# carrenD/Medical-Cross-Modality-Domain-Adaptation

Hardware: AMD Instinct MI355X
Metric: training slices/sec (256x256x3, B=16/GPU) joint segmenter+GAN step (1 dis update on B MR + B CT, clip, 1 gen update on B CT) (higher is better)
Workload: dtype f32; 1 GPU; BASELINE configs[3]: train_gan.py --phase train-gan joint step, B=16/GPU per domain, f32, dropout .75, mask critic on; global_batch=16, per_gpu_batch=16, parallelism=dp1, step_capture=False

## Files before the change

include/pnp_hip.h:

```cpp
#ifndef PNP_HIP_H
#define PNP_HIP_H

#include <stddef.h>
#include <stdint.h>

#ifdef __cplusplus
extern "C" {
#endif

#define PNP_OK 0
#define PNP_EINVAL (-1)
#define PNP_ELAUNCH (-2)
#define PNP_EWORKSPACE (-3)
#define PNP_ECOMM (-4)

#define PNP_DTYPE_F32 0
#define PNP_DTYPE_BF16 1
#define PNP_DTYPE_F64 2

#define PNP_PAD_ZERO 0
#define PNP_PAD_SYMMETRIC 1

int pnp_abi_version(void);
const char* pnp_last_error(void);
int pnp_device_info(int device, int* cu_count, int* clock_khz, int* lds_bytes, char* arch, int arch_len);

#define PNP_PROF_CONV_FWD 1
#define PNP_PROF_CONV_DGRAD 2
#define PNP_PROF_CONV_WGRAD 4
#define PNP_PROF_CONV_DIRECT 8
typedef struct pnp_prof_row {
    char name[128];
    int64_t launches;
    double ms, flops, bytes;
} pnp_prof_row;
int pnp_prof_enable(int32_t mask);
int pnp_prof_summary(pnp_prof_row* rows, int32_t max_rows);

typedef struct pnp_conv_geom {
    int32_t N, H, W, C;
    int32_t K, R, S;
    int32_t OH, OW;
    int32_t stride, dil;
    int32_t pad_t, pad_l;
    int32_t pad_mode;
    int32_t dtype;
} pnp_conv_geom;

int pnp_conv2d_fwd(const float* x, const float* w, float* y, const pnp_conv_geom* g,
                   float keep_prob, uint64_t seed, uint32_t stream_id, void* stream);
size_t pnp_conv2d_fwd_workspace_bytes(const pnp_conv_geom* g);
int pnp_conv2d_fwd_ws(const float* x, const float* w, float* y, const pnp_conv_geom* g,
                      float keep_prob, uint64_t seed, uint32_t stream_id,
                      void* workspace, size_t workspace_bytes, void* stream);

int32_t pnp_conv2d_fwd_stats_parts(const pnp_conv_geom* g);
int pnp_conv2d_fwd_stats(const float* x, const float* w, float* y, const pnp_conv_geom* g,
                         float keep_prob, uint64_t seed, uint32_t stream_id,
                         const float* shift , float* parts, size_t parts_bytes, void* stream);
int32_t pnp_conv2d_fwd_stats_ws_parts(const pnp_conv_geom* g);
int pnp_conv2d_fwd_stats_ws(const float* x, const float* w, float* y, const pnp_conv_geom* g,
                            float keep_prob, uint64_t seed, uint32_t stream_id,
                            const float* shift , float* parts, size_t parts_bytes,
// ... 245 lines not shown
```

medical-cross-modality-domain-adaptation_amd/_lib.py:

```python
import ctypes
import os

import torch

from ctypes import POINTER, c_char_p, c_float, c_int, c_int32, c_int64, c_size_t, c_uint32, c_uint64, c_void_p

_HERE = os.path.dirname(os.path.abspath(__file__))
LIB_PATH = os.environ.get("PNP_LIB") or os.path.join(_HERE, "libpnp_hip.so")

PAD_ZERO = 0
PAD_SYMMETRIC = 1
OPT_CHUNK = 1024
DTYPE_F32, DTYPE_BF16, DTYPE_F64 = 0, 1, 2
COMM_ID_BYTES = 128
(ROUTE_IGEMM, ROUTE_N16, ROUTE_NARROW, ROUTE_WINO, ROUTE_X3D, ROUTE_X3S, ROUTE_PHASES,
 ROUTE_WINO_WGRAD, ROUTE_X3W, ROUTE_N16_WGRAD, ROUTE_WGD, ROUTE_RING) = range(12)
ABI_VERSION = 4


class ConvGeom(ctypes.Structure):
    _fields_ = [(n, c_int32) for n in
                ("N", "H", "W", "C", "K", "R", "S", "OH", "OW", "stride", "dil", "pad_t", "pad_l", "pad_mode", "dtype")]

    def key(self):
        return tuple(getattr(self, f) for f, _ in self._fields_)


class ProfRow(ctypes.Structure):
    _fields_ = [("name", ctypes.c_char * 128), ("launches", c_int64), ("ms", ctypes.c_double), ("flops", ctypes.c_double),
                ("bytes", ctypes.c_double)]


class AugVolume(ctypes.Structure):
    _fields_ = [("image", c_void_p), ("label", c_void_p), ("X", c_int32), ("Y", c_int32), ("Z", c_int32), ("fill", c_float)]


class AugSample(ctypes.Structure):
    _fields_ = [("volume", c_int32), ("frame", c_int32), ("m", c_float * 6)]


class AugSampleZ(ctypes.Structure):
    _fields_ = [("volume", c_int32), ("frame", c_int32), ("dz", c_float), ("m", c_float * 6)]


PROF_CONV_FWD, PROF_CONV_DGRAD, PROF_CONV_WGRAD, PROF_CONV_DIRECT = 1, 2, 4, 8


class PnpError(RuntimeError):
    pass


_F = c_void_p
_G = POINTER(ConvGeom)

PROTOTYPES = {
    "pnp_abi_version": (c_int, []),
    "pnp_last_error": (c_char_p, []),
    "pnp_device_info": (c_int, [c_int, POINTER(c_int), POINTER(c_int), POINTER(c_int), c_char_p, c_int]),
    "pnp_prof_enable": (c_int, [c_int32]),
    "pnp_prof_summary": (c_int, [POINTER(ProfRow), c_int32]),
    "pnp_conv2d_fwd": (c_int, [_F, _F, _F, _G, c_float, c_uint64, c_uint32, c_void_p]),
    "pnp_conv2d_dgrad_workspace_bytes": (c_size_t, [_G]),
    "pnp_conv2d_dgrad": (c_int, [_F, _F, _F, _G, c_void_p, c_size_t, c_void_p]),
    "pnp_conv2d_dgrad_add": (c_int, [_F, _F, _F, _F, _G, c_void_p, c_size_t, c_void_p]),
    "pnp_conv2d_wgrad_workspace_bytes": (c_size_t, [_G]),
    "pnp_conv2d_wgrad": (c_int, [_F, _F, _F, _G, c_void_p, c_size_t, c_void_p]),
    "pnp_conv2d_wgrad_acc": (c_int, [_F, _F, _F, _G, c_void_p, c_size_t, c_void_p]),
    "pnp_conv2d_fwd_workspace_bytes": (c_size_t, [_G]),
    "pnp_conv2d_fwd_ws": (c_int, [_F, _F, _F, _G, c_float, c_uint64, c_uint32, c_void_p, c_size_t, c_void_p]),
    "pnp_conv2d_fwd_stats_parts": (c_int32, [_G]),
    "pnp_conv2d_fwd_stats": (c_int, [_F, _F, _F, _G, c_float, c_uint64, c_uint32, _F, _F, c_size_t, c_void_p]),
    "pnp_bn_stats_finish": (c_int, [_F, c_int32, _F, _F, _F, _F, _F, c_int64, c_int32, c_float, c_void_p]),
    "pnp_bn_fold": (c_int, [_F, _F, _F, _F, _F, _F, c_int32, c_float, c_void_p]),
    "pnp_conv2d_fwd_bn": (c_int, [_F, _F, _F, _G, c_float, c_uint64, c_uint32, _F, _F, _F, c_int32, c_float, c_void_p]),
    "pnp_conv2d_fwd_bn_ws": (c_int, [_F, _F, _F, _G, c_float, c_uint64, c_uint32, _F, _F, _F, c_int32, c_float, c_void_p, c_size_t, c_void_p]),
    "pnp_conv2d_fwd_stats_ws_parts": (c_int32, [_G]),
    "pnp_conv2d_fwd_stats_ws": (c_int, [_F, _F, _F, _G, c_float, c_uint64, c_uint32, _F, _F, c_size_t, c_void_p, c_size_t, c_void_p]),
    "pnp_conv2d_wino_chosen": (c_int32, [_G, c_int32]),
# ... 151 lines not shown
```

medical-cross-modality-domain-adaptation_amd/csrc/conv_wino.hip:

```cpp
#include <atomic>
#include <map>
#include <mutex>
#include "conv_common.h"
#include "conv_mma.h"

using namespace pnpconv;

namespace {

constexpr int NT = 256;

__device__ __forceinline__ f32x4 ld4(const float* p) { return *reinterpret_cast<const f32x4*>(p); }
__device__ __forceinline__ void st4(float* p, f32x4 v) { *reinterpret_cast<f32x4*>(p) = v; }

typedef __bf16 bf16x4 __attribute__((ext_vector_type(4)));
__device__ __forceinline__ void split3(float v, __bf16& hi, __bf16& mid, __bf16& lo) {
    hi = (__bf16)v;
    const float r = v - (float)hi;
    mid = (__bf16)r;
    lo = (__bf16)(r - (float)mid);
}
__device__ __forceinline__ void st4x3(__bf16* p, size_t pstride, f32x4 v) {
    bf16x4 h, m, l;
#pragma unroll
// ... 387 lines not shown
#pragma unroll
        for (int i = 0; i < NR; ++i) abase[i] = abase_n[i];
#pragma unroll
        for (int i = 0; i < NPB; ++i) boff[i] = boff_n[i];
        pos = pos_n; m0 = m0_n; n0 = n0_n;
        if (next_tail) in_tail = true;
        else local = nl;
    }
}

struct WinoOutArgs {
    const float* Mm;
    float* y;
    WinoGeom g;
    int K;
    int tiles_per_block;
    int do_drop;
    uint32_t drop_thresh, drop_key;
    float drop_keep;
    const pnp_step_params* sp;
    uint32_t drop_sid;
    const float* res_add;
    float* stat_ws;
    const float* stat_shift;
    const float* ep_scale;
    const float* ep_shift;
    const float* ep_res;
    int ep_cs;
    float ep_alpha;
    const float* Px;
    int tail_P, tail_F, tail_R, tail_s, tail_bn, nblk_m, nblk_n, gn;
};

template <int M, bool TS = false>
__global__ void __launch_bounds__(NT) wino_out_kernel(WinoOutArgs a) {
    constexpr int P = M + 2;
    __shared__ float red[NT * 8];
    const int K4 = a.K >> 2;
    const int kq0 = blockIdx.y * NT;
    const int K4s = (K4 - kq0) < NT ? (K4 - kq0) : NT;
    const int rpi = NT / K4s;
    const int tid = threadIdx.x;
    const int cg = tid % K4s, rsub = tid / K4s;
    const bool active = rsub < rpi;
    const int k = (kq0 + cg) * 4;
    const int t0 = blockIdx.x * a.tiles_per_block;
    int t1 = t0 + a.tiles_per_block;
    if (t1 > a.g.T) t1 = a.g.T;
    const size_t plane = (size_t)a.g.T * a.K;
    const uint32_t dkey = a.do_drop ? pnp_eff_drop_key(a.drop_key, a.sp, a.drop_sid) : 0u;
    const bool stats = a.stat_ws != nullptr;
    f32x4 s0 = {0, 0, 0, 0}, s1 = {0, 0, 0, 0};
    if (active) {
        f32x4 shift = {0, 0, 0, 0}, sc = {0, 0, 0, 0}, sh = {0, 0, 0, 0};
        if (stats && a.stat_shift) shift = ld4(a.stat_shift + k);
        if (a.ep_scale) {
            sc = ld4(a.ep_scale + k);
            sh = ld4(a.ep_shift + k);
        }
        const int cpad = (a.K - a.ep_cs) >> 1;
        for (int t = t0 + rsub; t < t1; t += rpi) {
            int n, pa, pb, ti, tj;
            tile_of(a.g, t, n, pa, pb, ti, tj);
            const float* src = a.Mm + (size_t)t * a.K + k;
            f32x4 m[P][P];
#pragma unroll
            for (int p = 0; p < P; ++p)
#pragma unroll
                for (int q = 0; q < P; ++q) m[p][q] = ld4(src + (size_t)(P * p + q) * plane);
            if constexpr (TS) {
                const int mt = t >> 7, nt = k / a.tail_bn;
                int bid;
                if (a.gn <= 0 || a.gn >= a.nblk_n) bid = mt * a.nblk_n + nt;
                else {
                    const int sc = nt / a.gn, left = a.nblk_n - sc * a.gn;
                    const int width = left < a.gn ? left : a.gn;
                    bid = sc * (a.nblk_m * a.gn) + mt * width + (nt - sc * a.gn);
                }
                const int nblk = a.nblk_m * a.nblk_n;
                int x = bid / a.tail_P, local = bid - x * a.tail_P;
                const size_t tsz = (size_t)128 * a.tail_bn;
                const size_t inner = (size_t)(t & 127) * a.tail_bn + (k - nt * a.tail_bn);
#pragma unroll
                for (int p = 0; p < P; ++p)
#pragma unroll
                    for (int q = 0; q < P; ++q) {
                        if (local >= a.tail_F) {
                            const float* px = a.Px + (size_t)(x * a.tail_R + local - a.tail_F) * (a.tail_s - 1) * tsz + inner;
                            for (int pc = 0; pc < a.tail_s - 1; ++pc) m[p][q] += ld4(px + pc * tsz);
                        }
                        local += nblk;
                        if (local >= a.tail_P) {
                            local -= a.tail_P;
                            ++x;
                        }
                    }
            }
            f32x4 o[M][M];
            if constexpr (M == 2) {
                f32x4 r[2][4];
#pragma unroll
                for (int q = 0; q < 4; ++q) {
                    r[0][q] = m[0][q] + m[1][q] + m[2][q];
                    r[1][q] = m[1][q] - m[2][q] - m[3][q];
                }
#pragma unroll
                for (int p = 0; p < 2; ++p) {
                    o[p][0] = r[p][0] + r[p][1] + r[p][2];
                    o[p][1] = r[p][1] - r[p][2] - r[p][3];
                }
            } else {
                f32x4 r[4][6];
#pragma unroll
                for (int q = 0; q < 6; ++q) {
                    f32x4 c4[4];
                    w4_at(m[0][q], m[1][q], m[2][q], m[3][q], m[4][q], m[5][q], c4);
#pragma unroll
                    for (int p = 0; p < 4; ++p) r[p][q] = c4[p];
                }
#pragma unroll
                for (int p = 0; p < 4; ++p) w4_at(r[p][0], r[p][1], r[p][2], r[p][3], r[p][4], r[p][5], o[p]);
            }
#pragma unroll
            for (int p = 0; p < M; ++p)
#pragma unroll
                for (int q = 0; q < M; ++q) {
                    const int u = M * ti + p, v = M * tj + q;
                    if (u >= a.g.Hso || v >= a.g.Wso) continue;
                    const size_t row = (size_t)(n * a.g.Ho + pa + a.g.dil * u) * a.g.Wo + pb + a.g.dil * v;
                    const size_t idx = row * a.K + k;
                    f32x4 val = o[p][q];
                    if (a.do_drop) {
#pragma unroll
                        for (int e = 0; e < 4; ++e)
                            val[e] = pnp_drop_keep((uint32_t)(idx + e), dkey, a.drop_thresh) ? val[e] / a.drop_keep : 0.f;
                    }
                    if (a.res_add) val += ld4(a.res_add + idx);
                    if (stats) {
#pragma unroll
                        for (int e = 0; e < 4; ++e) {
                            const float d = val[e] - shift[e];
                            s0[e] += d;
                            s1[e] = fmaf(d, d, s1[e]);
                        }
                    }
                    if (a.ep_scale) {
#pragma unroll
                        for (int e = 0; e < 4; ++e) val[e] = fmaf(val[e], sc[e], sh[e]);
                        if (a.ep_res) {
#pragma unroll
                            for (int e = 0; e < 4; ++e) {
                                const int cs = k + e - cpad;
                                if ((unsigned)cs < (unsigned)a.ep_cs) val[e] += a.ep_res[row * a.ep_cs + cs];
                            }
                        }
                        if (a.ep_alpha >= 0.f) {
#pragma unroll
                            for (int e = 0; e < 4; ++e) val[e] = val[e] < 0.f ? val[e] * a.ep_alpha : val[e];
                        }
                    }
                    st4(a.y + idx, val);
                }
        }
    }
    if (!stats) return;
#pragma unroll
    for (int e = 0; e < 4; ++e) {
        red[tid * 8 + e] = s0[e];
        red[tid * 8 + 4 + e] = s1[e];
    }
    __syncthreads();
    if (tid < K4s) {
        f32x4 a0 = {0, 0, 0, 0}, a1 = {0, 0, 0, 0};
        for (int j = 0; j < rpi; ++j) {
            const int tt = j * K4s + tid;
#pragma unroll
            for (int e = 0; e < 4; ++e) {
                a0[e] += red[tt * 8 + e];
                a1[e] += red[tt * 8 + 4 + e];
            }
        }
        st4(a.stat_ws + ((size_t)blockIdx.x * 2 + 0) * a.K + k, a0);
        st4(a.stat_ws + ((size_t)blockIdx.x * 2 + 1) * a.K + k, a1);
    }
}


struct WinoDyArgs {
    const float* dy;
    float* Y;
    WinoGeom g;
    int K;
};

template <int M>
__global__ void __launch_bounds__(NT) wino_dy_kernel(WinoDyArgs a) {
    const int K4 = a.K >> 2;
    const size_t nvec = (size_t)a.g.T * K4;
    const size_t plane = (size_t)a.g.T * a.K;
    const size_t gs = (size_t)gridDim.x * NT;
    for (size_t i = (size_t)blockIdx.x * NT + threadIdx.x; i < nvec; i += gs) {
        const int t = (int)(i / K4);
        const int k = (int)(i - (size_t)t * K4) * 4;
        int n, pa, pb, ti, tj;
        tile_of(a.g, t, n, pa, pb, ti, tj);
        f32x4 y[M][M];
#pragma unroll
        for (int p = 0; p < M; ++p)
#pragma unroll
            for (int q = 0; q < M; ++q) {
                const int u = M * ti + p, v = M * tj + q;
                const f32x4 zero = {0, 0, 0, 0};
                y[p][q] = (u < a.g.Hso && v < a.g.Wso) ? ld4(a.dy + ((size_t)(n * a.g.Ho + pa + a.g.dil * u) * a.g.Wo + pb + a.g.dil * v) * a.K + k) : zero;
            }
        float* out = a.Y + (size_t)t * a.K + k;
        if constexpr (M == 2) {
// ... 639 lines not shown
        ga.V = V; ga.U = U; ga.Mm = Mm; ga.T = w.T; ga.C = a.C; ga.K = a.K;
        const bool narrow = a.K <= 64;
        ga.nblk_m = pnp_cdiv(w.T, 128); ga.nblk_n = pnp_cdiv(a.K, narrow ? 64 : 128);
        static const int wino_gn = env_int("PNP_WINO_GN", -1);
        ga.gn = wino_gn >= 0 ? wino_gn : a.gn; ga.xcd_swizzle = xcd ? 2 : 0;
        ga.npos = NP;
        ga.whole = ((double)NP * w.T * a.C * 4.0 < 2147483648.0 && (double)NP * a.C * a.K * 4.0 < 2147483648.0) ? 1 : 0;
        ga.tail_F = plan.F; ga.tail_R = plan.R; ga.tail_s = plan.s; ga.Px = Px;
        dim3 grid((unsigned)plan.grid);
        const double fl = 2.0 * NP * (double)w.T * a.C * a.K;
        const double by = 4.0 * NP * ((double)w.T * a.C + (double)a.C * a.K + (double)w.T * a.K);
        constexpr int KB = M == 4 ? 2 : 0;
        PnpProfScope ps(cls, st, fl, by, "wino_gemm_kernel<128, %d, 2, 2, %d>", narrow ? 64 : 128, KB + (kind != 0));
        if (narrow) {
            if (kind == 0) hipLaunchKernelGGL((wino_gemm_kernel<128, 64, 2, 2, KB>), grid, dim3(NTHREADS), 0, st, ga);
            else hipLaunchKernelGGL((wino_gemm_kernel<128, 64, 2, 2, KB + 1>), grid, dim3(NTHREADS), 0, st, ga);
        } else if (kind == 0) hipLaunchKernelGGL((wino_gemm_kernel<128, 128, 2, 2, KB>), grid, dim3(NTHREADS), 0, st, ga);
        else hipLaunchKernelGGL((wino_gemm_kernel<128, 128, 2, 2, KB + 1>), grid, dim3(NTHREADS), 0, st, ga);
        PNP_CHECK_LAUNCH("wino_gemm_kernel");
    }
    {
        WinoOutArgs oa{};
        oa.Mm = Mm; oa.y = a.y; oa.g = w; oa.K = a.K;
        int nblk;
        out_plan(w.T, a.K, &oa.tiles_per_block, &nblk);
        oa.do_drop = a.do_drop; oa.drop_thresh = a.drop_thresh; oa.drop_key = a.drop_key; oa.drop_keep = a.drop_keep;
        oa.sp = a.sp; oa.drop_sid = a.drop_sid;
        oa.res_add = a.res_add; oa.stat_ws = a.stat_ws; oa.stat_shift = a.stat_shift;
        oa.ep_scale = a.ep_scale; oa.ep_shift = a.ep_shift; oa.ep_res = a.ep_res; oa.ep_cs = a.ep_cs; oa.ep_alpha = a.ep_alpha;
        oa.Px = Px; oa.tail_P = plan.P; oa.tail_F = plan.F; oa.tail_R = plan.R; oa.tail_s = plan.s; oa.tail_bn = a.K <= 64 ? 64 : 128;
        static const int wino_gn_o = env_int("PNP_WINO_GN", -1);
        oa.nblk_m = pnp_cdiv(w.T, 128); oa.nblk_n = pnp_cdiv(a.K, oa.tail_bn); oa.gn = wino_gn_o >= 0 ? wino_gn_o : a.gn;
        dim3 grid((unsigned)nblk, (unsigned)pnp_cdiv(a.K / 4, NT));
        PnpProfScope ps(cls, st, 0.0, 4.0 * ((double)NP * w.T * a.K + (double)a.M * a.K), "wino_out_kernel<%d>", M);
        if (oa.tail_s > 1) hipLaunchKernelGGL((wino_out_kernel<M, true>), grid, dim3(NT), 0, st, oa);
        else hipLaunchKernelGGL((wino_out_kernel<M, false>), grid, dim3(NT), 0, st, oa);
        PNP_CHECK_LAUNCH("wino_out_kernel");
    }
    return PNP_OK;
}

int launch_wino(const ConvArgs& a, int kind, bool flip_transpose, void* ws, size_t ws_bytes, hipStream_t st) {
    const int m = plan_tile(a, false);
    PNP_REQUIRE(m == 2 || m == 4, "launch_wino: the planner does not route this layer (policy changed between the query and the launch?)");
    return m == 4 ? launch_wino_m<4>(a, kind, flip_transpose, ws, ws_bytes, st) : launch_wino_m<2>(a, kind, flip_transpose, ws, ws_bytes, st);
}

int wino_wgrad_tile(const pnp_conv_geom* g) { return plan_tile(g, true); }

inline int x3_tp(int T) { return (T + 63) & ~63; }
inline bool use_x3_wgrad(int T, int C, int K) {
    static const int on = env_int("PNP_WINOGRAD_X3_WGRAD", 1), tmin = env_int("PNP_WINOGRAD_X3_WGRAD_TMIN", 256), tmax = env_int("PNP_WINOGRAD_X3_WGRAD_TMAX", 2048);
    const int m = wino_x3_mode();
    if (!on || m == 0 || !wino_x3_dims_ok(C, x3_tp(T), K) || !wino_x3_dims_ok(K, x3_tp(T), C)) return false;
    return m >= 2 || (T >= tmin && T <= tmax);
}
int wgrad_split_x3(int T, int C, int K, int npos, int* sps) {
    const int nchunks = x3_tp(T) / 64;
    const long long tiles = (long long)pnp_cdiv(C, 128) * pnp_cdiv(K, K <= 64 ? 64 : 128) * npos;
    int best = 1;
    double best_cost = 1e30;
    for (int ns = 1; ns <= 32 && ns <= nchunks; ++ns) {
        const int cps = pnp_cdiv(nchunks, ns);
        if (pnp_cdiv(nchunks, cps) != ns) continue;
        if (ns > 1 && cps < 2) break;
        const int rounds = pnp_cdiv(tiles * ns, 256);
        const double cost = rounds * (2.0 * cps + 3.0) + ns * 1.5e-6 * npos * (double)C * K;
        if (cost < best_cost - 1e-9) { best_cost = cost; best = ns; }
    }
// ... 189 lines not shown
```

medical-cross-modality-domain-adaptation_amd/csrc/elementwise.hip:

```cpp
#include <atomic>
#include <mutex>
#include "pnp_common.h"

namespace {

constexpr int NT = 256;

__device__ __forceinline__ f32x4 ld4(const float* p) { return *reinterpret_cast<const f32x4*>(p); }
__device__ __forceinline__ void st4(float* p, f32x4 v) { *reinterpret_cast<f32x4*>(p) = v; }
typedef __bf16 bf16x4_t __attribute__((ext_vector_type(4)));
__device__ __forceinline__ void st4h(__bf16* p, f32x4 v) {
    bf16x4_t h;
    h[0] = (__bf16)v[0]; h[1] = (__bf16)v[1]; h[2] = (__bf16)v[2]; h[3] = (__bf16)v[3];
    *reinterpret_cast<bf16x4_t*>(p) = h;
}

inline dim3 grid_rows(long long P, int C4, int cap = 256 * 8) {
    const int ny = (C4 + NT - 1) / NT;
    const int c4s = C4 < NT ? C4 : NT;
    const int rpi = NT / c4s;
    long long bx = (P + rpi - 1) / rpi;
    const long long cx = cap / ny > 0 ? cap / ny : 1;
    if (bx > cx) bx = cx;
    if (bx < 1) bx = 1;
// ... 2 lines not shown

inline int grid_for(size_t nvec, int cap = 256 * 8) {
    long long b = (long long)((nvec + NT - 1) / NT);
    if (b > cap) b = cap;
    if (b < 1) b = 1;
    return (int)b;
}

struct ColArgs {
    const float* x;
    const float* dout;
    const float* out;
    const float* mean;
    const float* var;
    const float* gamma;
    const float* beta;
    float* ws;
    long long P;
    int C;
    int rows_per_block;
    float eps, alpha;
    unsigned* tick;
    int nslab;
    float* o0;
    float* o1;
    float* acc0;
    float* acc1;
    float* mm;
    float* mv;
    float decay;
};

constexpr int COLRED_SLAB = 128;

template <int KIND>
__global__ void __launch_bounds__(NT) colreduce_kernel(ColArgs a) {
    __shared__ float red[NT * 8];
    __shared__ int s_last;
    const int C4 = a.C >> 2;
    const int rpi = NT / C4;
    const int t = threadIdx.x;
    const int cg = t % C4, rsub = t / C4;
    const bool active = rsub < rpi;
    const long long r0 = (long long)blockIdx.x * a.rows_per_block;
    long long r1 = r0 + a.rows_per_block;
    if (r1 > a.P) r1 = a.P;
    f32x4 s0 = {0, 0, 0, 0}, s1 = {0, 0, 0, 0};
    if (active) {
        const int c = cg * 4;
        f32x4 m, rs, gsc = {0, 0, 0, 0}, bet = {0, 0, 0, 0};
        if constexpr (KIND == 0) {
            m = ld4(a.x + c);
        } else {
            m = ld4(a.mean + c);
            f32x4 v = ld4(a.var + c);
#pragma unroll
            for (int e = 0; e < 4; ++e) rs[e] = 1.0f / sqrtf(v[e] + a.eps);
            if (!a.out && a.alpha >= 0.f) {
                const f32x4 ga = ld4(a.gamma + c);
                bet = ld4(a.beta + c);
#pragma unroll
                for (int e = 0; e < 4; ++e) gsc[e] = ga[e] * rs[e];
            }
        }
        for (long long r = r0 + rsub; r < r1; r += rpi) {
            const size_t off = (size_t)r * a.C + c;
            f32x4 xv = ld4(a.x + off);
            if constexpr (KIND == 0) {
#pragma unroll
                for (int e = 0; e < 4; ++e) {
                    float d = xv[e] - m[e];
                    s0[e] += d;
                    s1[e] = fmaf(d, d, s1[e]);
                }
            } else {
                f32x4 g = ld4(a.dout + off);
                if (a.alpha >= 0.f) {
                    if (a.out) {
                        f32x4 o = ld4(a.out + off);
#pragma unroll
                        for (int e = 0; e < 4; ++e) g[e] = o[e] > 0.f ? g[e] : g[e] * a.alpha;
                    } else {
#pragma unroll
                        for (int e = 0; e < 4; ++e) g[e] = fmaf(xv[e] - m[e], gsc[e], bet[e]) > 0.f ? g[e] : g[e] * a.alpha;
                    }
                }
#pragma unroll
                for (int e = 0; e < 4; ++e) {
                    float xh = (xv[e] - m[e]) * rs[e];
                    s0[e] += g[e];
                    s1[e] = fmaf(g[e], xh, s1[e]);
                }
            }
        }
    }
#pragma unroll
    for (int e = 0; e < 4; ++e) {
        red[t * 8 + e] = s0[e];
        red[t * 8 + 4 + e] = s1[e];
    }
    __syncthreads();
    if (t < C4) {
        f32x4 a0 = {0, 0, 0, 0}, a1 = {0, 0, 0, 0};
        for (int j = 0; j < rpi; ++j) {
            const int tt = j * C4 + t;
#pragma unroll
            for (int e = 0; e < 4; ++e) {
                a0[e] += red[tt * 8 + e];
                a1[e] += red[tt * 8 + 4 + e];
            }
        }
        float* w0 = a.ws + ((size_t)blockIdx.x * 2 + 0) * a.C + t * 4;
        float* w1 = a.ws + ((size_t)blockIdx.x * 2 + 1) * a.C + t * 4;
        st4(w0, a0);
        st4(w1, a1);
    }
    if (!a.tick) return;
    const int nblk = (int)gridDim.x;
    const int slab = blockIdx.x / COLRED_SLAB;
    const int b0 = slab * COLRED_SLAB;
    const int b1 = (b0 + COLRED_SLAB < nblk) ? b0 + COLRED_SLAB : nblk;
    __threadfence();
    __syncthreads();
    if (t == 0) s_last = (atomicAdd(&a.tick[slab], 1u) == (unsigned)(b1 - b0 - 1));
    __syncthreads();
    if (!s_last) return;
    __threadfence();
    double* dred = reinterpret_cast<double*>(red);
    double d0[4] = {0, 0, 0, 0}, d1[4] = {0, 0, 0, 0};
    if (active) {
        for (int b = b0 + rsub; b < b1; b += rpi) {
            const f32x4 v0 = ld4(a.ws + ((size_t)b * 2 + 0) * a.C + cg * 4), v1 = ld4(a.ws + ((size_t)b * 2 + 1) * a.C + cg * 4);
#pragma unroll
            for (int e = 0; e < 4; ++e) {
                d0[e] += (double)v0[e];
                d1[e] += (double)v1[e];
            }
        }
    }
    double t0[4] = {0, 0, 0, 0}, t1[4] = {0, 0, 0, 0};
#pragma unroll
    for (int q = 0; q < 2; ++q) {
// ... 164 lines not shown
        s1 += red[1][j][cl];
    }
    if constexpr (KIND == 0) {
        const double inv = 1.0 / (double)P;
        const double md = s0 * inv;
        double var = s1 * inv - md * md;
        if (var < 0.0) var = 0.0;
        const float meanf = (float)((double)x0[c] + md), varf = (float)var;
        o0[c] = meanf;
        o1[c] = varf;
        if (mm) {
            const float one_minus = 1.0f - decay;
            const float bessel = P > 1 ? (float)((double)P / (double)(P - 1)) : 1.0f;
            mm[c] -= (mm[c] - meanf) * one_minus;
            mv[c] -= (mv[c] - varf * bessel) * one_minus;
        }
    } else {
        o0[c] = (float)s0;
        o1[c] = (float)s1;
        if (acc0) {
            acc0[c] += (float)s0;
            acc1[c] += (float)s1;
        }
    }
}

template <int KIND>
int launch_colreduce_final(float* ws, const float* x0, float* o0, float* o1, int nblk, int C, long long P, float* mm, float* mv, float decay,
                           hipStream_t st, const char* who, float* acc0 = nullptr, float* acc1 = nullptr) {
    static const int two_stage = getenv("PNP_BN_FINAL_1STAGE") ? 0 : 1;
    int slab = 0, n = nblk;
    if (two_stage && nblk >= 4 * COLRED_SLAB) {
        const int nslab = nblk / COLRED_SLAB;
        hipLaunchKernelGGL(colreduce_compact_kernel, dim3(pnp_cdiv(C, 32), nslab), dim3(1024), 0, st, ws, nblk, nslab, C);
        PNP_CHECK_LAUNCH(who);
        slab = COLRED_SLAB;
        n = 2 * nslab;
    }
    hipLaunchKernelGGL(colreduce_final_kernel<KIND>, dim3(pnp_cdiv(C, 32)), dim3(1024), 0, st, (const float*)ws, x0, o0, o1, n, C, P, mm, mv,
                       decay, slab, acc0, acc1);
    PNP_CHECK_LAUNCH(who);
    return PNP_OK;
}

int colreduce_plan(long long P, int C, int* nblk, int* rpb) {
    static const int cap = getenv("PNP_BN_NBLK") ? atoi(getenv("PNP_BN_NBLK")) : 2048;
    long long b = (P + 63) / 64;
    if (b > cap) b = cap;
    if (b < 1) b = 1;
    long long r = (P + b - 1) / b;
    b = (P + r - 1) / r;
    *nblk = (int)b;
    *rpb = (int)r;
    (void)C;
    return 0;
}

constexpr int TICKET_SLOTS = 512, TICKET_STRIDE = 32;
unsigned* ticket_slot(hipStream_t st, int nslab) {
    static const int on = getenv("PNP_BN_ONE_LAUNCH") ? atoi(getenv("PNP_BN_ONE_LAUNCH")) : 0;
    if (!on || nslab + 1 > TICKET_STRIDE) return nullptr;
    constexpr int MAXDEV = 16;
    static std::atomic<unsigned*> bufs[MAXDEV];
    static std::atomic<unsigned> seq{0};
    static std::mutex mx;
    int dev = 0;
    if (hipGetDevice(&dev) != hipSuccess || dev < 0 || dev >= MAXDEV) {
        (void)hipGetLastError();
        return nullptr;
    }
    std::atomic<unsigned*>& buf = bufs[dev];
    unsigned* b = buf.load(std::memory_order_acquire);
    if (!b) {
        hipStreamCaptureStatus cs = hipStreamCaptureStatusNone;
        if (hipStreamIsCapturing(st, &cs) != hipSuccess || cs != hipStreamCaptureStatusNone) {
            (void)hipGetLastError();
            return nullptr;
        }
        std::lock_guard<std::mutex> lk(mx);
        b = buf.load(std::memory_order_acquire);
        if (!b) {
            if (hipMalloc((void**)&b, sizeof(unsigned) * TICKET_SLOTS * TICKET_STRIDE) != hipSuccess ||
                hipMemset(b, 0, sizeof(unsigned) * TICKET_SLOTS * TICKET_STRIDE) != hipSuccess || hipDeviceSynchronize() != hipSuccess) {
                (void)hipGetLastError();
                return nullptr;
            }
            buf.store(b, std::memory_order_release);
        }
    }
    return b + (size_t)(seq.fetch_add(1, std::memory_order_relaxed) % TICKET_SLOTS) * TICKET_STRIDE;
}

template <int KIND>
int run_colreduce(ColArgs a, float* o0, float* o1, void* ws, size_t ws_bytes, hipStream_t st, const char* who, float* mm = nullptr,
                  float* mv = nullptr, float decay = 0.f, float* acc0 = nullptr, float* acc1 = nullptr) {
    int nblk, rpb;
    colreduce_plan(a.P, a.C, &nblk, &rpb);
    const size_t need = (size_t)nblk * 2 * a.C * sizeof(float);
    if (ws_bytes < need || !ws) {
        pnp_set_error("%s: workspace too small (%zu < %zu)", who, ws_bytes, need);
        return PNP_EWORKSPACE;
    }
    a.ws = (float*)ws;
    a.rows_per_block = rpb;
    if ((a.C & 3) == 0 && a.C <= 1024) {
        a.nslab = pnp_cdiv(nblk, COLRED_SLAB);
        a.tick = ticket_slot(st, a.nslab);
        a.o0 = o0; a.o1 = o1; a.acc0 = acc0; a.acc1 = acc1; a.mm = mm; a.mv = mv; a.decay = decay;
        hipLaunchKernelGGL(colreduce_kernel<KIND>, dim3(nblk), dim3(NT), 0, st, a);
        if (a.tick) {
            PNP_CHECK_LAUNCH(who);
            return PNP_OK;
        }
    } else {
        hipLaunchKernelGGL(colreduce_scalar_kernel<KIND>, dim3(nblk, pnp_cdiv(a.C, 64)), dim3(64), 0, st, a);
    }
    PNP_CHECK_LAUNCH(who);
    return launch_colreduce_final<KIND>((float*)ws, a.x, o0, o1, nblk, a.C, a.P, mm, mv, decay, st, who, acc0, acc1);
}

__global__ void bn_update_moving_kernel(float* mm, float* mv, const float* mean, const float* var, long long P, int C,
                                        float decay) {
    const int c = blockIdx.x * blockDim.x + threadIdx.x;
    if (c >= C) return;
    const float one_minus = 1.0f - decay;
    const float bessel = P > 1 ? (float)((double)P / (double)(P - 1)) : 1.0f;
    mm[c] -= (mm[c] - mean[c]) * one_minus;
    mv[c] -= (mv[c] - var[c] * bessel) * one_minus;
}

struct BnApplyArgs {
    const float *x, *mean, *var, *gamma, *beta, *shortcut;
    float* y;
    long long P;
    int C, Cs;
    float eps, alpha;
    __bf16* yh;
};

template <bool VEC>
__global__ void __launch_bounds__(NT) bn_apply_kernel(BnApplyArgs a) {
    const int cpad = (a.C - a.Cs) / 2;
// ... 409 lines not shown
};
__global__ void __launch_bounds__(NT) critic_input_bwd_kernel(CriticBwdArgs k) {
    const int Csrc = k.Ca + k.Cb + k.Cc + k.Cd + k.ncls;
    const size_t total = (size_t)k.P * Csrc;
    const size_t gs = (size_t)gridDim.x * NT;
    const int o1 = k.Ca * k.tile_a, o2 = o1 + k.Cb, o3 = o2 + k.Cc, o4 = o3 + k.Cd;
    for (size_t i = (size_t)blockIdx.x * NT + threadIdx.x; i < total; i += gs) {
        const size_t p = i / Csrc;
        int ch = (int)(i - p * Csrc);
        const float* g = k.dout + p * k.Ctot;
        if (ch < k.Ca) {
            float s = 0.f;
            for (int t = 0; t < k.tile_a; ++t) s += g[t * k.Ca + ch];
            if (k.da) k.da[p * k.Ca + ch] = s;
            continue;
        }
        ch -= k.Ca;
        if (ch < k.Cb) { if (k.db) k.db[p * k.Cb + ch] = g[o1 + ch]; continue; }
        ch -= k.Cb;
        if (ch < k.Cc) { if (k.dc) k.dc[p * k.Cc + ch] = g[o2 + ch]; continue; }
        ch -= k.Cc;
        if (ch < k.Cd) { if (k.dd) k.dd[p * k.Cd + ch] = g[o3 + ch]; continue; }
        ch -= k.Cd;
        if (k.dlogits) k.dlogits[p * k.ncls + ch] = g[o4 + ch];
    }
}

}

extern "C" {

size_t pnp_bn_workspace_bytes(int64_t P, int32_t C) {
    int nblk, rpb;
    colreduce_plan(P, C, &nblk, &rpb);
    return (size_t)nblk * 2 * C * sizeof(float);
}

int pnp_bn_stats(const float* x, float* mean, float* var, int64_t P, int32_t C, void* workspace, size_t workspace_bytes,
                 void* stream) {
    PNP_REQUIRE(x && mean && var && P > 0 && C > 0, "pnp_bn_stats: bad argument");
    ColArgs a{};
    a.x = x; a.P = P; a.C = C;
    return run_colreduce<0>(a, mean, var, workspace, workspace_bytes, (hipStream_t)stream, "pnp_bn_stats");
}

int pnp_bn_stats_update(const float* x, float* mean, float* var, float* moving_mean, float* moving_var, int64_t P, int32_t C, float decay,
                        void* workspace, size_t workspace_bytes, void* stream) {
    PNP_REQUIRE(x && mean && var && moving_mean && moving_var && P > 0 && C > 0, "pnp_bn_stats_update: bad argument");
    ColArgs a{};
    a.x = x; a.P = P; a.C = C;
    return run_colreduce<0>(a, mean, var, workspace, workspace_bytes, (hipStream_t)stream, "pnp_bn_stats_update", moving_mean, moving_var, decay);
}

int pnp_bn_stats_finish(float* parts, int32_t nparts, const float* shift, float* mean, float* var, float* moving_mean,
                        float* moving_var, int64_t P, int32_t C, float decay, void* stream) {
    PNP_REQUIRE(parts && shift && mean && var && nparts > 0 && P > 0 && C > 0, "pnp_bn_stats_finish: bad argument");
    PNP_REQUIRE((moving_mean != nullptr) == (moving_var != nullptr), "pnp_bn_stats_finish: moving_mean and moving_var go together");
    return launch_colreduce_final<0>(parts, shift, mean, var, nparts, C, (long long)P, moving_mean, moving_var, decay, (hipStream_t)stream,
                                     "pnp_bn_stats_finish");
}

int pnp_bn_update_moving(float* moving_mean, float* moving_var, const float* mean, const float* var, int64_t P, int32_t C,
                         float decay, void* stream) {
    PNP_REQUIRE(moving_mean && moving_var && mean && var && P > 0 && C > 0, "pnp_bn_update_moving: bad argument");
    hipLaunchKernelGGL(bn_update_moving_kernel, dim3(pnp_cdiv(C, 64)), dim3(64), 0, (hipStream_t)stream, moving_mean,
                       moving_var, mean, var, (long long)P, C, decay);
    PNP_CHECK_LAUNCH("pnp_bn_update_moving");
// ... 204 lines not shown
```

Baseline: 291.4 slices/s.

## Retune Winograd output and BN column-reduce kernels for bandwidth and occupancy

The Winograd output transform now uses 2-wide vectors for M=4, which doubles the thread count. It loads through buffer resources with scalar offsets, specializes on the epilogue and large-tensor cases, and sets waves-per-EU hints. The BN column-reduce kernel moves to 512 threads with a 4-row unrolled load loop and a transposed shared-memory layout that avoids bank conflicts. Its block-count plan is also reworked so the grid stays under the two-stage compaction threshold. Profiling scopes are added for the BN reduce kernels. The risks are register pressure from the unrolling, different reduction ordering, and workspace sizing that now depends on kind while the workspace query always passes 0.

```diff
diff --git a/include/pnp_hip.h b/include/pnp_hip.h
--- a/include/pnp_hip.h
+++ b/include/pnp_hip.h
@@ -29,6 +29,7 @@
 #define PNP_PROF_CONV_DGRAD 2
 #define PNP_PROF_CONV_WGRAD 4
 #define PNP_PROF_CONV_DIRECT 8
+#define PNP_PROF_BN_REDUCE 16
 typedef struct pnp_prof_row {
     char name[128];
     int64_t launches;
diff --git a/medical-cross-modality-domain-adaptation_amd/_lib.py b/medical-cross-modality-domain-adaptation_amd/_lib.py
--- a/medical-cross-modality-domain-adaptation_amd/_lib.py
+++ b/medical-cross-modality-domain-adaptation_amd/_lib.py
@@ -44,6 +44,7 @@
 
 
 PROF_CONV_FWD, PROF_CONV_DGRAD, PROF_CONV_WGRAD, PROF_CONV_DIRECT = 1, 2, 4, 8
+PROF_BN_REDUCE = 16
 
 
 class PnpError(RuntimeError):
diff --git a/medical-cross-modality-domain-adaptation_amd/csrc/conv_wino.hip b/medical-cross-modality-domain-adaptation_amd/csrc/conv_wino.hip
--- a/medical-cross-modality-domain-adaptation_amd/csrc/conv_wino.hip
+++ b/medical-cross-modality-domain-adaptation_amd/csrc/conv_wino.hip
@@ -443,42 +443,71 @@
     int tail_P, tail_F, tail_R, tail_s, tail_bn, nblk_m, nblk_n, gn;
 };
 
-template <int M, bool TS = false>
-__global__ void __launch_bounds__(NT) wino_out_kernel(WinoOutArgs a) {
+constexpr int wino_out_vw(int m) { return m == 4 ? 2 : 4; }
+constexpr int wino_out_nt(int m) { return NT * 4 / wino_out_vw(m); }
+
+template <int M, bool TS = false, bool EP = false, bool BIG = false>
+__global__ void __launch_bounds__(wino_out_nt(M)) __attribute__((amdgpu_waves_per_eu(TS || EP || BIG ? 1 : 4))) wino_out_kernel(WinoOutArgs a) {
     constexpr int P = M + 2;
-    __shared__ float red[NT * 8];
-    const int K4 = a.K >> 2;
+    constexpr int VW = wino_out_vw(M);
+    constexpr int NT = wino_out_nt(M);
+    typedef float V __attribute__((ext_vector_type(VW)));
+    auto ldv = [](const float* p) { return *reinterpret_cast<const V*>(p); };
+    auto bldv = [](__amdgpu_buffer_rsrc_t r, unsigned off, int soff) {
+        if constexpr (VW == 2) return __builtin_bit_cast(V, __builtin_amdgcn_raw_buffer_load_b64(r, off, soff, 0));
+        else return __builtin_bit_cast(V, __builtin_amdgcn_raw_buffer_load_b128(r, off, soff, 0));
+    };
+    __shared__ float red[2 * VW * NT];
+    const int K4 = a.K / VW;
     const int kq0 = blockIdx.y * NT;
     const int K4s = (K4 - kq0) < NT ? (K4 - kq0) : NT;
     const int rpi = NT / K4s;
     const int tid = threadIdx.x;
     const int cg = tid % K4s, rsub = tid / K4s;
     const bool active = rsub < rpi;
-    const int k = (kq0 + cg) * 4;
+    const int k = (kq0 + cg) * VW;
     const int t0 = blockIdx.x * a.tiles_per_block;
     int t1 = t0 + a.tiles_per_block;
     if (t1 > a.g.T) t1 = a.g.T;
     const size_t plane = (size_t)a.g.T * a.K;
+    const int pbytes = BIG ? 0 : (int)(plane * 4);
+    const __amdgpu_buffer_rsrc_t rm = make_rsrc(a.Mm, BIG ? 0u : (unsigned)(plane * 4 * P * P));
     const uint32_t dkey = a.do_drop ? pnp_eff_drop_key(a.drop_key, a.sp, a.drop_sid) : 0u;
     const bool stats = a.stat_ws != nullptr;
-    f32x4 s0 = {0, 0, 0, 0}, s1 = {0, 0, 0, 0};
+    V s0 = 0.f, s1 = 0.f;
     if (active) {
-        f32x4 shift = {0, 0, 0, 0}, sc = {0, 0, 0, 0}, sh = {0, 0, 0, 0};
-        if (stats && a.stat_shift) shift = ld4(a.stat_shift + k);
-        if (a.ep_scale) {
-            sc = ld4(a.ep_scale + k);
-            sh = ld4(a.ep_shift + k);
+        V shift = 0.f, sc = 0.f, sh = 0.f;
+        if (stats && a.stat_shift) shift = ldv(a.stat_shift + k);
+        if (EP && a.ep_scale) {
+            sc = ldv(a.ep_scale + k);
+            sh = ldv(a.ep_shift + k);
         }
         const int cpad = (a.K - a.ep_cs) >> 1;
         for (int t = t0 + rsub; t < t1; t += rpi) {
-            int n, pa, pb, ti, tj;
-            tile_of(a.g, t, n, pa, pb, ti, tj);
-            const float* src = a.Mm + (size_t)t * a.K + k;
-            f32x4 m[P][P];
-#pragma unroll
-            for (int p = 0; p < P; ++p)
-#pragma unroll
-                for (int q = 0; q < P; ++q) m[p][q] = ld4(src + (size_t)(P * p + q) * plane);
+            unsigned tu = (unsigned)t;
+            const int tj = (int)(tu % (unsigned)a.g.tw);
+            tu /= (unsigned)a.g.tw;
+            const int ti = (int)(tu % (unsigned)a.g.th);
+            tu /= (unsigned)a.g.th;
+            const int dsh = a.g.dil >> 1, dmask = a.g.dil - 1;
+            const int pb = (int)tu & dmask, pa = (int)(tu >> dsh) & dmask, n = (int)(tu >> (2 * dsh));
+            V m[P][P];
+            if constexpr (BIG) {
+                const float* src = a.Mm + (size_t)t * a.K + k;
+#pragma unroll
+                for (int p = 0; p < P; ++p)
+#pragma unroll
+                    for (int q = 0; q < P; ++q) m[p][q] = ldv(src + (size_t)(P * p + q) * plane);
+            } else {
+                constexpr int QG = P / 2;
+                unsigned voff[2];
+#pragma unroll
+                for (int h = 0; h < 2; ++h) voff[h] = (unsigned)(t * a.K + k) * 4u + (unsigned)(h * QG * pbytes);
+#pragma unroll
+                for (int p = 0; p < P; ++p)
+#pragma unroll
+                    for (int q = 0; q < P; ++q) m[p][q] = bldv(rm, voff[q / QG], (P * p + q % QG) * pbytes);
+            }
             if constexpr (TS) {
                 const int mt = t >> 7, nt = k / a.tail_bn;
                 int bid;
@@ -498,7 +527,7 @@
                     for (int q = 0; q < P; ++q) {
                         if (local >= a.tail_F) {
                             const float* px = a.Px + (size_t)(x * a.tail_R + local - a.tail_F) * (a.tail_s - 1) * tsz + inner;
-                            for (int pc = 0; pc < a.tail_s - 1; ++pc) m[p][q] += ld4(px + pc * tsz);
+                            for (int pc = 0; pc < a.tail_s - 1; ++pc) m[p][q] += ldv(px + pc * tsz);
                         }
                         local += nblk;
                         if (local >= a.tail_P) {
@@ -507,9 +536,9 @@
                         }
                     }
             }
-            f32x4 o[M][M];
+            V o[M][M];
             if constexpr (M == 2) {
-                f32x4 r[2][4];
+                V r[2][4];
 #pragma unroll
                 for (int q = 0; q < 4; ++q) {
                     r[0][q] = m[0][q] + m[1][q] + m[2][q];
@@ -521,10 +550,10 @@
                     o[p][1] = r[p][1] - r[p][2] - r[p][3];
                 }
             } else {
-                f32x4 r[4][6];
+                V r[4][6];
 #pragma unroll
                 for (int q = 0; q < 6; ++q) {
-                    f32x4 c4[4];
+                    V c4[4];
                     w4_at(m[0][q], m[1][q], m[2][q], m[3][q], m[4][q], m[5][q], c4);
 #pragma unroll
                     for (int p = 0; p < 4; ++p) r[p][q] = c4[p];
@@ -532,6 +561,7 @@
 #pragma unroll
                 for (int p = 0; p < 4; ++p) w4_at(r[p][0], r[p][1], r[p][2], r[p][3], r[p][4], r[p][5], o[p]);
             }
+            __builtin_amdgcn_sched_barrier(0);
 #pragma unroll
             for (int p = 0; p < M; ++p)
 #pragma unroll
@@ -540,59 +570,59 @@
                     if (u >= a.g.Hso || v >= a.g.Wso) continue;
                     const size_t row = (size_t)(n * a.g.Ho + pa + a.g.dil * u) * a.g.Wo + pb + a.g.dil * v;
                     const size_t idx = row * a.K + k;
-                    f32x4 val = o[p][q];
+                    V val = o[p][q];
                     if (a.do_drop) {
 #pragma unroll
-                        for (int e = 0; e < 4; ++e)
+                        for (int e = 0; e < VW; ++e)
                             val[e] = pnp_drop_keep((uint32_t)(idx + e), dkey, a.drop_thresh) ? val[e] / a.drop_keep : 0.f;
                     }
-                    if (a.res_add) val += ld4(a.res_add + idx);
+                    if (a.res_add) val += ldv(a.res_add + idx);
                     if (stats) {
 #pragma unroll
-                        for (int e = 0; e < 4; ++e) {
+                        for (int e = 0; e < VW; ++e) {
                             const float d = val[e] - shift[e];
                             s0[e] += d;
                             s1[e] = fmaf(d, d, s1[e]);
                         }
                     }
-                    if (a.ep_scale) {
-#pragma unroll
-                        for (int e = 0; e < 4; ++e) val[e] = fmaf(val[e], sc[e], sh[e]);
+                    if (EP && a.ep_scale) {
+#pragma unroll
+                        for (int e = 0; e < VW; ++e) val[e] = fmaf(val[e], sc[e], sh[e]);
                         if (a.ep_res) {
 #pragma unroll
-                            for (int e = 0; e < 4; ++e) {
+                            for (int e = 0; e < VW; ++e) {
                                 const int cs = k + e - cpad;
                                 if ((unsigned)cs < (unsigned)a.ep_cs) val[e] += a.ep_res[row * a.ep_cs + cs];
                             }
                         }
                         if (a.ep_alpha >= 0.f) {
 #pragma unroll
-                            for (int e = 0; e < 4; ++e) val[e] = val[e] < 0.f ? val[e] * a.ep_alpha : val[e];
+                            for (int e = 0; e < VW; ++e) val[e] = val[e] < 0.f ? val[e] * a.ep_alpha : val[e];
                         }
                     }
-                    st4(a.y + idx, val);
+                    *reinterpret_cast<V*>(a.y + idx) = val;
                 }
         }
     }
     if (!stats) return;
 #pragma unroll
-    for (int e = 0; e < 4; ++e) {
-        red[tid * 8 + e] = s0[e];
-        red[tid * 8 + 4 + e] = s1[e];
+    for (int e = 0; e < VW; ++e) {
+        red[e * NT + tid] = s0[e];
+        red[(VW + e) * NT + tid] = s1[e];
     }
     __syncthreads();
     if (tid < K4s) {
-        f32x4 a0 = {0, 0, 0, 0}, a1 = {0, 0, 0, 0};
+        V a0 = 0.f, a1 = 0.f;
         for (int j = 0; j < rpi; ++j) {
             const int tt = j * K4s + tid;
 #pragma unroll
-            for (int e = 0; e < 4; ++e) {
-                a0[e] += red[tt * 8 + e];
-                a1[e] += red[tt * 8 + 4 + e];
-            }
-        }
-        st4(a.stat_ws + ((size_t)blockIdx.x * 2 + 0) * a.K + k, a0);
-        st4(a.stat_ws + ((size_t)blockIdx.x * 2 + 1) * a.K + k, a1);
+            for (int e = 0; e < VW; ++e) {
+                a0[e] += red[e * NT + tt];
+                a1[e] += red[(VW + e) * NT + tt];
+            }
+        }
+        *reinterpret_cast<V*>(a.stat_ws + ((size_t)blockIdx.x * 2 + 0) * a.K + k) = a0;
+        *reinterpret_cast<V*>(a.stat_ws + ((size_t)blockIdx.x * 2 + 1) * a.K + k) = a1;
     }
 }
 
@@ -1298,9 +1328,14 @@
         static const int wino_gn_o = env_int("PNP_WINO_GN", -1);
         oa.nblk_m = pnp_cdiv(w.T, 128); oa.nblk_n = pnp_cdiv(a.K, oa.tail_bn); oa.gn = wino_gn_o >= 0 ? wino_gn_o : a.gn;
         dim3 grid((unsigned)nblk, (unsigned)pnp_cdiv(a.K / 4, NT));
+        const dim3 ont(wino_out_nt(M));
         PnpProfScope ps(cls, st, 0.0, 4.0 * ((double)NP * w.T * a.K + (double)a.M * a.K), "wino_out_kernel<%d>", M);
-        if (oa.tail_s > 1) hipLaunchKernelGGL((wino_out_kernel<M, true>), grid, dim3(NT), 0, st, oa);
-        else hipLaunchKernelGGL((wino_out_kernel<M, false>), grid, dim3(NT), 0, st, oa);
+        const bool big = (double)NP * w.T * a.K * 4.0 >= 2147483648.0;
+        if (oa.tail_s > 1 && !big) hipLaunchKernelGGL((wino_out_kernel<M, true, true, false>), grid, ont, 0, st, oa);
+        else if (oa.tail_s > 1) hipLaunchKernelGGL((wino_out_kernel<M, true, true, true>), grid, ont, 0, st, oa);
+        else if (big) hipLaunchKernelGGL((wino_out_kernel<M, false, true, true>), grid, ont, 0, st, oa);
+        else if (oa.ep_scale) hipLaunchKernelGGL((wino_out_kernel<M, false, true, false>), grid, ont, 0, st, oa);
+        else hipLaunchKernelGGL((wino_out_kernel<M, false, false, false>), grid, ont, 0, st, oa);
         PNP_CHECK_LAUNCH("wino_out_kernel");
     }
     return PNP_OK;
diff --git a/medical-cross-modality-domain-adaptation_amd/csrc/elementwise.hip b/medical-cross-modality-domain-adaptation_amd/csrc/elementwise.hip
--- a/medical-cross-modality-domain-adaptation_amd/csrc/elementwise.hip
+++ b/medical-cross-modality-domain-adaptation_amd/csrc/elementwise.hip
@@ -58,9 +58,11 @@
 };
 
 constexpr int COLRED_SLAB = 128;
+constexpr int CR_NT = 512, CR_U = 4;
 
 template <int KIND>
-__global__ void __launch_bounds__(NT) colreduce_kernel(ColArgs a) {
+__global__ void __launch_bounds__(CR_NT) colreduce_kernel(ColArgs a) {
+    constexpr int NT = CR_NT;
     __shared__ float red[NT * 8];
     __shared__ int s_last;
     const int C4 = a.C >> 2;
@@ -89,9 +91,9 @@
                 for (int e = 0; e < 4; ++e) gsc[e] = ga[e] * rs[e];
             }
         }
-        for (long long r = r0 + rsub; r < r1; r += rpi) {
-            const size_t off = (size_t)r * a.C + c;
-            f32x4 xv = ld4(a.x + off);
+        const bool use_out = KIND == 1 && a.alpha >= 0.f && a.out;
+        const f32x4 zero = {0, 0, 0, 0};
+        auto add_row = [&](const f32x4& xv, f32x4 g, const f32x4& o) {
             if constexpr (KIND == 0) {
 #pragma unroll
                 for (int e = 0; e < 4; ++e) {
@@ -100,10 +102,8 @@
                     s1[e] = fmaf(d, d, s1[e]);
                 }
             } else {
-                f32x4 g = ld4(a.dout + off);
                 if (a.alpha >= 0.f) {
                     if (a.out) {
-                        f32x4 o = ld4(a.out + off);
 #pragma unroll
                         for (int e = 0; e < 4; ++e) g[e] = o[e] > 0.f ? g[e] : g[e] * a.alpha;
                     } else {
@@ -118,12 +118,28 @@
                     s1[e] = fmaf(g[e], xh, s1[e]);
                 }
             }
-        }
+        };
+        long long r = r0 + rsub;
+        const size_t step = (size_t)rpi * a.C;
+        size_t off = (size_t)r * a.C + c;
+        for (; r + (long long)(CR_U - 1) * rpi < r1; r += (long long)CR_U * rpi, off += CR_U * step) {
+            f32x4 xv[CR_U], g[CR_U], o[CR_U];
+#pragma unroll
+            for (int u = 0; u < CR_U; ++u) {
+                xv[u] = ld4(a.x + off + u * step);
+                g[u] = KIND == 1 ? ld4(a.dout + off + u * step) : zero;
+                o[u] = use_out ? ld4(a.out + off + u * step) : zero;
+            }
+#pragma unroll
+            for (int u = 0; u < CR_U; ++u) add_row(xv[u], g[u], o[u]);
+        }
+        for (; r < r1; r += rpi, off += step)
+            add_row(ld4(a.x + off), KIND == 1 ? ld4(a.dout + off) : zero, use_out ? ld4(a.out + off) : zero);
     }
 #pragma unroll
     for (int e = 0; e < 4; ++e) {
-        red[t * 8 + e] = s0[e];
-        red[t * 8 + 4 + e] = s1[e];
+        red[e * NT + t] = s0[e];
+        red[(4 + e) * NT + t] = s1[e];
     }
     __syncthreads();
     if (t < C4) {
@@ -132,8 +148,8 @@
             const int tt = j * C4 + t;
 #pragma unroll
             for (int e = 0; e < 4; ++e) {
-                a0[e] += red[tt * 8 + e];
-                a1[e] += red[tt * 8 + 4 + e];
+                a0[e] += red[e * NT + tt];
+                a1[e] += red[(4 + e) * NT + tt];
             }
         }
         float* w0 = a.ws + ((size_t)blockIdx.x * 2 + 0) * a.C + t * 4;
@@ -364,27 +380,40 @@
     int slab = 0, n = nblk;
     if (two_stage && nblk >= 4 * COLRED_SLAB) {
         const int nslab = nblk / COLRED_SLAB;
+        PnpProfScope ps(PNP_PROF_BN_REDUCE, st, 0.0, 8.0 * nblk * C, "colreduce_compact_kernel");
         hipLaunchKernelGGL(colreduce_compact_kernel, dim3(pnp_cdiv(C, 32), nslab), dim3(1024), 0, st, ws, nblk, nslab, C);
         PNP_CHECK_LAUNCH(who);
         slab = COLRED_SLAB;
         n = 2 * nslab;
     }
+    PnpProfScope ps(PNP_PROF_BN_REDUCE, st, 0.0, 8.0 * n * C, "colreduce_final_kernel<%d>", KIND);
     hipLaunchKernelGGL(colreduce_final_kernel<KIND>, dim3(pnp_cdiv(C, 32)), dim3(1024), 0, st, (const float*)ws, x0, o0, o1, n, C, P, mm, mv,
                        decay, slab, acc0, acc1);
     PNP_CHECK_LAUNCH(who);
     return PNP_OK;
 }
 
-int colreduce_plan(long long P, int C, int* nblk, int* rpb) {
-    static const int cap = getenv("PNP_BN_NBLK") ? atoi(getenv("PNP_BN_NBLK")) : 2048;
-    long long b = (P + 63) / 64;
-    if (b > cap) b = cap;
+int colreduce_plan(long long P, int C, int kind, int* nblk, int* rpb) {
+    static const int cap_env = getenv("PNP_BN_NBLK") ? atoi(getenv("PNP_BN_NBLK")) : 0;
+    const bool vec = (C & 3) == 0 && C <= 1024;
+    long long b, r;
+    if (vec) {
+        const int cap = cap_env > 0 ? cap_env : 4 * COLRED_SLAB - 1;
+        const int rpi = CR_NT / (C >> 2);
+        long long iters = (P + (long long)rpi * cap - 1) / ((long long)rpi * cap);
+        if (iters < 1) iters = 1;
+        r = iters * rpi;
+    } else {
+        const int cap = cap_env > 0 ? cap_env : (kind == 0 ? 2048 : 4 * COLRED_SLAB - 1);
+        b = (P + 63) / 64;
+        if (b > cap) b = cap;
+        if (b < 1) b = 1;
+        r = (P + b - 1) / b;
+    }
+    b = (P + r - 1) / r;
     if (b < 1) b = 1;
-    long long r = (P + b - 1) / b;
-    b = (P + r - 1) / r;
     *nblk = (int)b;
     *rpb = (int)r;
-    (void)C;
     return 0;
 }
 
@@ -427,7 +456,7 @@
 int run_colreduce(ColArgs a, float* o0, float* o1, void* ws, size_t ws_bytes, hipStream_t st, const char* who, float* mm = nullptr,
                   float* mv = nullptr, float decay = 0.f, float* acc0 = nullptr, float* acc1 = nullptr) {
     int nblk, rpb;
-    colreduce_plan(a.P, a.C, &nblk, &rpb);
+    colreduce_plan(a.P, a.C, KIND, &nblk, &rpb);
     const size_t need = (size_t)nblk * 2 * a.C * sizeof(float);
     if (ws_bytes < need || !ws) {
         pnp_set_error("%s: workspace too small (%zu < %zu)", who, ws_bytes, need);
@@ -435,11 +464,14 @@
     }
     a.ws = (float*)ws;
     a.rows_per_block = rpb;
+    const double tensors = KIND == 0 ? 1.0 : (a.out && a.alpha >= 0.f ? 3.0 : 2.0);
+    PnpProfScope ps(PNP_PROF_BN_REDUCE, st, 0.0, 4.0 * tensors * (double)a.P * a.C, "%s<%d>",
+                    ((a.C & 3) == 0 && a.C <= 1024) ? "colreduce_kernel" : "colreduce_scalar_kernel", KIND);
     if ((a.C & 3) == 0 && a.C <= 1024) {
         a.nslab = pnp_cdiv(nblk, COLRED_SLAB);
         a.tick = ticket_slot(st, a.nslab);
         a.o0 = o0; a.o1 = o1; a.acc0 = acc0; a.acc1 = acc1; a.mm = mm; a.mv = mv; a.decay = decay;
-        hipLaunchKernelGGL(colreduce_kernel<KIND>, dim3(nblk), dim3(NT), 0, st, a);
+        hipLaunchKernelGGL(colreduce_kernel<KIND>, dim3(nblk), dim3(CR_NT), 0, st, a);
         if (a.tick) {
             PNP_CHECK_LAUNCH(who);
             return PNP_OK;
@@ -915,7 +947,7 @@
 
 size_t pnp_bn_workspace_bytes(int64_t P, int32_t C) {
     int nblk, rpb;
-    colreduce_plan(P, C, &nblk, &rpb);
+    colreduce_plan(P, C, 0, &nblk, &rpb);
     return (size_t)nblk * 2 * C * sizeof(float);
 }
 
```

After: 293.9 slices/s, median of 6. About the same (+0.9%).
